# SuhailSama/MR_RL

Measured on NVIDIA B200. Metric: env_steps_per_sec, higher is better.
Workload: dtype f64

## Files before the change

mr_rl_b200/csrc/mr_api.cu:

```cuda
#include <cstdarg>
#include <cstdio>
#include <cstdlib>
#include <initializer_list>
#include <new>

#include "mr_common.cuh"

namespace mr {

thread_local char g_err[512] = "";

static int step_path_from_env() {
    const char* e = getenv("MR_STEP_PATH");
    if (!e) return 0;
    if (e[0] == 't' && e[1] == 'm' && e[2] == 'a' && e[3] == 'p') return 5;
    return e[0] == 't' ? 1 : e[0] == 'v' ? 2 : e[0] == 's' ? 3 : e[0] == 'w' ? 4 : 0;
}
int g_step_path = step_path_from_env();
thread_local int g_step_cta_cap = 0;
static int actor_path_from_env() {
    const char* e = getenv("MR_ACTOR_PATH");
    return !e ? 0 : e[0] == 's' ? 1 : e[0] == 't' ? 2 : 0;
}
int g_actor_path = actor_path_from_env();
// ... 388 lines not shown
            return mr::fail(MR_ERR_ARG, "mr_env_step_host: direct mode shares one row stride between obs_host and state_prime");
        oh.skip_goal_rows = io->copy_goal_rows ? 0 : 1;
        oh.out_f32 = io->io_f32 ? 1 : 0;
        mr_sim_params ph = *p;
        if (io->io_f32) { ph.action_f32 = 1; oh.state_prime = nullptr; }
        mr::g_step_cta_cap = 1;
        rc = mr_env_step(st, n, dtype, &ph, nz, tt, io->actions_host, &oh, stream);
        mr::g_step_cta_cap = 0;
        if (rc) return rc;
        const cudaError_t e0 = cudaStreamSynchronize((cudaStream_t)stream);
        if (e0 != cudaSuccess) return mr::fail(MR_ERR_CUDA, "mr_env_step_host: %s", cudaGetErrorString(e0));
        return MR_OK;
    }
    if (!pl || !out_dev) return mr::fail(MR_ERR_ARG, "mr_env_step_host: staged mode needs a pipeline and device output rows");
    const bool zc_in = io->actions_dev == nullptr;
    if (!out_dev->obs || !out_dev->rew || !out_dev->done) return mr::fail(MR_ERR_ARG, "mr_env_step_host: device obs/rew/done rows required");
    const int64_t dstride = out_dev->row_stride ? out_dev->row_stride : n;
    int chunks = n_chunks < 1 ? 1 : (n_chunks > pl->max_chunks ? pl->max_chunks : n_chunks);
    if (nz && nz->mode == MR_NOISE_TABLE) chunks = 1;
    int64_t per = (n / chunks) / 256 * 256;
    if (per == 0) { chunks = 1; per = n; }
    cudaStream_t cur = (cudaStream_t)stream;
    cudaError_t ce = cudaSuccess;
    auto ok = [&](cudaError_t r) { if (ce == cudaSuccess && r != cudaSuccess) ce = r; return ce == cudaSuccess; };
    ok(cudaEventRecord(pl->ev_start, cur));
    ok(cudaStreamWaitEvent(pl->s_in, pl->ev_start, 0));
    ok(cudaStreamWaitEvent(pl->s_k, pl->ev_start, 0));
    ok(cudaStreamWaitEvent(pl->s_out, pl->ev_start, 0));
    for (int c = 0; c < chunks && ce == cudaSuccess && rc == MR_OK; ++c) {
        const int64_t lo = c * per, hi = c == chunks - 1 ? n : lo + per, m = hi - lo;
        if (!zc_in) {
            if (!ok(cudaMemcpyAsync((char*)io->actions_dev + 2 * lo * el, (const char*)io->actions_host + 2 * lo * el,
                                    (size_t)(2 * m * el), cudaMemcpyHostToDevice, pl->s_in))) break;
            if (!ok(cudaEventRecord(pl->ev_in[c], pl->s_in)) || !ok(cudaStreamWaitEvent(pl->s_k, pl->ev_in[c], 0))) break;
        }
        mr_env_state sc = *st;
        sc.x = (char*)st->x + lo * el; sc.y = (char*)st->y + lo * el; sc.fx = (char*)st->fx + lo * el;
        sc.fy = (char*)st->fy + lo * el; sc.h = (char*)st->h + lo * el;
        sc.counter = st->counter + lo; sc.status = st->status + lo;
        if (st->cursor) sc.cursor = st->cursor + lo;
        mr_step_out oc = *out_dev;
        oc.obs = (char*)out_dev->obs + lo * el; oc.rew = (char*)out_dev->rew + lo * el; oc.done = out_dev->done + lo;
        if (out_dev->state_prime) oc.state_prime = (char*)out_dev->state_prime + lo * el;
        oc.row_stride = dstride;
        mr_noise nc;
        const mr_noise* nzp = nz;
        if (nz) { nc = *nz; nc.env_base = nz->env_base + (uint64_t)lo; nzp = &nc; }
        rc = mr_env_step(&sc, m, dtype, p, nzp, tt, (const char*)(zc_in ? io->actions_host : io->actions_dev) + 2 * lo * el, &oc,
                         pl->s_k);
        if (rc) break;
        if (!ok(cudaEventRecord(pl->ev_k[c], pl->s_k)) || !ok(cudaStreamWaitEvent(pl->s_out, pl->ev_k[c], 0))) break;
        ok(cudaMemcpy2DAsync((char*)io->obs_host + lo * el, (size_t)(hstride * el), (const char*)out_dev->obs + lo * el,
                             (size_t)(dstride * el), (size_t)(m * el), io->copy_goal_rows ? 4 : 2, cudaMemcpyDeviceToHost, pl->s_out));
        ok(cudaMemcpyAsync((char*)io->obs_host + (4 * hstride + lo) * el, (const char*)out_dev->obs + (4 * dstride + lo) * el,
                           (size_t)(m * el), cudaMemcpyDeviceToHost, pl->s_out));
        if (io->rew_host)
            ok(cudaMemcpyAsync((char*)io->rew_host + lo * el, (const char*)out_dev->rew + lo * el, (size_t)(m * el),
// ... 72 lines not shown
```

mr_rl_b200/csrc/mr_step_tma.cuh:

```cuda
#pragma once

#include "mr_common.cuh"

namespace mr {

#ifndef MR_STAGES_IN
#define MR_STAGES_IN 3
#endif
#ifdef MR_TILE
template <class T> struct TileOf { static constexpr int value = MR_TILE; };
#else
template <class T> struct TileOf { static constexpr int value = sizeof(T) == 8 ? 128 : 256; };
#endif
constexpr int kStagesIn = MR_STAGES_IN;
constexpr int kStagesOut = 2;

__device__ __forceinline__ uint32_t smem_u32(const void* p) { return (uint32_t)__cvta_generic_to_shared(p); }

__device__ __forceinline__ void mbar_init(uint64_t* bar, uint32_t count) {
    asm volatile("mbarrier.init.shared::cta.b64 [%0], %1;" ::"r"(smem_u32(bar)), "r"(count));
}
__device__ __forceinline__ void mbar_expect_tx(uint64_t* bar, uint32_t bytes) {
    asm volatile("mbarrier.arrive.expect_tx.shared::cta.b64 _, [%0], %1;" ::"r"(smem_u32(bar)), "r"(bytes) : "memory");
}
// ... 42 lines not shown
__device__ __forceinline__ void bulk_commit() { asm volatile("cp.async.bulk.commit_group;" ::: "memory"); }
template <int N>
__device__ __forceinline__ void bulk_wait_read() { asm volatile("cp.async.bulk.wait_group.read %0;" ::"n"(N) : "memory"); }
__device__ __forceinline__ void fence_async_smem() { asm volatile("fence.proxy.async.shared::cta;" ::: "memory"); }

template <class T, int kTile>
struct alignas(128) TileIn {
    T x[kTile], y[kTile], fx[kTile], fy[kTile], h[kTile];
    T act[2 * kTile];
    int32_t counter[kTile];
};

template <class T, int kTile>
struct alignas(128) TileOut {
    T x[kTile], y[kTile], fx[kTile], fy[kTile], h[kTile];
    T d[kTile], rew[kTile], spx[kTile], spy[kTile];
    int32_t counter[kTile];
    uint8_t done[kTile];
};

template <int MODE, bool MISM> struct NoiseRows { static constexpr int value = 0; };
template <bool MISM> struct NoiseRows<MR_NOISE_TABLE, MISM> { static constexpr int value = MISM ? 24 : 16; };
template <int MODE> struct StagesIn { static constexpr int value = MODE == MR_NOISE_TABLE ? 2 : kStagesIn; };
#ifndef MR_ONE_BARRIER
#define MR_ONE_BARRIER 1
#endif
template <class T, int MODE> struct OneBarrier {
    static constexpr bool value = MR_ONE_BARRIER && (MODE == MR_NOISE_PHILOX || (MODE == MR_NOISE_NONE && sizeof(T) == 4));
};
template <class T, int MODE> struct StagesOut { static constexpr int value = OneBarrier<T, MODE>::value ? 3 : kStagesOut; };

template <int kTile, int ROWS>
struct alignas(128) TileNoiseIn {
    double z[ROWS][kTile];
// ... 24 lines not shown
    }
};

#ifndef MR_RNG_PREFETCH
#define MR_RNG_PREFETCH 0
#endif

template <class T, int MODE = MR_NOISE_NONE, bool MISM = false, int kTile = TileOf<T>::value>
struct StepSmem {
    static constexpr int kIn = StagesIn<MODE>::value;
    TileIn<T, kTile> in[kIn];
    static constexpr int kOut = StagesOut<T, MODE>::value;
    TileOut<T, kTile> out[kOut];
    TileNoiseIn<kTile, NoiseRows<MODE, MISM>::value> nin[kIn];
    TileNoiseOut<kTile, NoiseRows<MODE, MISM>::value> nout[kOut];
    alignas(128) T zero[2 * kTile];
    alignas(16) float4 zpre[(MR_RNG_PREFETCH && MODE == MR_NOISE_PHILOX && !MISM) ? 2 * kTile : 1];
    alignas(8) uint64_t full[kIn];
};

#ifndef MR_TMA_WARPS
#define MR_TMA_WARPS 16
#endif
#ifndef MR_TMA_WARPS_F32
#define MR_TMA_WARPS_F32 24
#endif
template <class T> struct TmaWarps { static constexpr int value = sizeof(T) == 4 ? MR_TMA_WARPS_F32 : MR_TMA_WARPS; };
template <class T, int MODE> struct TmaMinCtas {
    static constexpr int value = MODE == MR_NOISE_TABLE ? 1 : TmaWarps<T>::value * 32 / TileOf<T>::value;
};

template <class T, int MODE, bool MISM, bool TMAP>
__global__ void __launch_bounds__(TileOf<T>::value, TmaMinCtas<T, MODE>::value)
env_step_tma_kernel(StateView<T> st, const T* __restrict__ actions, OutView<T> out, NoiseView nv, TimeView tv,
                    Params p, int64_t n_tiles, int64_t n_total, const __grid_constant__ StepMaps maps) {
    constexpr int kTile = TileOf<T>::value;
    constexpr int kSI = StagesIn<MODE>::value;
    constexpr int kNR = NoiseRows<MODE, MISM>::value;
    constexpr bool kTable = MODE == MR_NOISE_TABLE;
    constexpr bool kOneBar = OneBarrier<T, MODE>::value;
    constexpr int kSO = StagesOut<T, MODE>::value;
    extern __shared__ __align__(128) unsigned char smem_raw[];
    using Smem = StepSmem<T, MODE, MISM>;
    Smem& sm = *reinterpret_cast<Smem*>(smem_raw);
    const int tid = threadIdx.x;
    const int64_t first = blockIdx.x, stride = gridDim.x;

    if (tid == 0) {
        for (int s = 0; s < kSI; ++s) mbar_init(&sm.full[s], 1);
        asm volatile("fence.mbarrier_init.release.cluster;" ::: "memory");
    }
    sm.zero[tid] = (T)0; sm.zero[kTile + tid] = (T)0;
    fence_async_smem();
    __syncthreads();
    asm volatile("griddepcontrol.launch_dependents;" ::: "memory");
    asm volatile("griddepcontrol.wait;" ::: "memory");

    constexpr uint32_t kRow = kTile * sizeof(T);
    const bool act32 = sizeof(T) == 8 && p.act_f32;
    const bool out32 = sizeof(T) == 8 && out.f32;
    const uint32_t act_bytes = act32 ? kTile * 8u : 2u * kRow;
    const uint32_t kInBytes = 5 * kRow + act_bytes + kTile * 4;
    const uint64_t off = step_offset(nv);

#ifndef MR_ISSUE_WARPS
#define MR_ISSUE_WARPS 1
#endif
    constexpr int kWarps = MR_ISSUE_WARPS;
    const int warp = tid >> 5;
    const bool elect = (tid & 31) == 0 && warp < kWarps;
    auto issue_loads = [&](int s, int64_t tile, int32_t cbase) {
        const int64_t i0 = tile * kTile;
        uint64_t* bar = &sm.full[s];
        TileIn<T, kTile>& b = sm.in[s];
        if constexpr (kTable) {
            int64_t rows = nv.table_len - (int64_t)cbase;
            rows = rows < 0 ? 0 : (rows > kNR ? kNR : rows);
            if (cbase < 0) rows = 0;
            sm.nin[s].base = cbase; sm.nin[s].rows = (int32_t)rows;
            if constexpr (TMAP) {
                mbar_expect_tx(bar, kInBytes + kTile * 4 + (uint32_t)kNR * kTile * 8);
                tensor_load_2d(sm.nin[s].z, &maps.table, (int32_t)i0, cbase < 0 ? 0 : cbase, bar);
            } else {
                mbar_expect_tx(bar, kInBytes + kTile * 4 + (uint32_t)rows * kTile * 8);
                const double* src = nv.table + (int64_t)cbase * nv.table_stride + nv.table_col0 + i0;
                for (int k = 0; k < (int)rows; ++k) bulk_load(sm.nin[s].z[k], src + (int64_t)k * nv.table_stride, kTile * 8, bar);
            }
// ... 3 lines not shown
        }
        if constexpr (TMAP) {
            tensor_load_2d(b.x, &maps.state, (int32_t)i0, 0, bar);
        } else {
            if (warp == 0 % kWarps) bulk_load(b.x, st.x + i0, kRow, bar);
            if (warp == 1 % kWarps) bulk_load(b.y, st.y + i0, kRow, bar);
            if (warp == 2 % kWarps) bulk_load(b.fx, st.fx + i0, kRow, bar);
            if (warp == 3 % kWarps) bulk_load(b.fy, st.fy + i0, kRow, bar);
            if (warp == 4 % kWarps) bulk_load(b.h, st.h + i0, kRow, bar);
        }
        if (warp == 5 % kWarps)
            bulk_load(b.act, act32 ? (const void*)(reinterpret_cast<const float*>(actions) + 2 * i0) : (const void*)(actions + 2 * i0),
                      act_bytes, bar);
        if (warp == 6 % kWarps) bulk_load(b.counter, st.counter + i0, kTile * 4, bar);
    };
    auto tile_cursor = [&](int64_t tile) -> int32_t {
        if constexpr (kTable) { if (tile < n_tiles) return st.cursor[tile * kTile]; }
        return 0;
    };

    int32_t cb_next = 0;
    if (elect) {
        for (int s = 0; s < kSI; ++s) {
            const int64_t tile = first + (int64_t)s * stride;
            if (tile < n_tiles) issue_loads(s, tile, tile_cursor(tile));
        }
        cb_next = tile_cursor(first + (int64_t)kSI * stride);
    }

    constexpr bool kPrefetch = MR_RNG_PREFETCH && MODE == MR_NOISE_PHILOX && !MISM;
    auto predraw = [&](int64_t tile) {
        if constexpr (kPrefetch) {
            PhiloxNoise nzp;
            nzp.seek(nv.env_base + (uint64_t)(tile * kTile + tid), off);
            float z8[8];
            nzp.draw8(p, z8);
            sm.zpre[tid] = make_float4(z8[0], z8[1], z8[2], z8[3]);
            sm.zpre[kTile + tid] = make_float4(z8[4], z8[5], z8[6], z8[7]);
        }
    };
    if (first < n_tiles) predraw(first);

    int it = 0;
    for (int64_t tile = first; tile < n_tiles; tile += stride, ++it) {
        const int s = it % kSI;
        const uint32_t parity = (uint32_t)(it / kSI) & 1u;
        const int so = it % kSO;
        const int64_t i0 = tile * kTile;

        mbar_wait(&sm.full[s], parity);
        Env e;
        const TileIn<T, kTile>& bi = sm.in[s];
        e.x = (double)bi.x[tid]; e.y = (double)bi.y[tid]; e.fx = (double)bi.fx[tid]; e.fy = (double)bi.fy[tid];
        const T h_raw = bi.h[tid];
        e.counter = bi.counter[tid]; e.status = 0; e.spx = e.spy = 0.0;
        double f_t, al;
        if (sizeof(T) == 8 && !act32) { const double2 a2 = reinterpret_cast<const double2*>(bi.act)[tid]; f_t = a2.x; al = a2.y; }
        else { const float2 a2 = reinterpret_cast<const float2*>(bi.act)[tid]; f_t = a2.x; al = a2.y; }

        if constexpr (!kOneBar) {
            if (elect) bulk_wait_read<kStagesOut - 1>();
            __syncthreads();
            if constexpr (!kTable) {
                if (elect) {
                    const int64_t nxt = tile + (int64_t)kSI * stride;
                    if (nxt < n_tiles) issue_loads(s, nxt, 0);
                }
            }
        }

        const double t = time_at(tv, e.counter, p.dt);
        const double tb = t + p.dt, tb2 = tb + p.dt;
        e.h = decode_h<T>(h_raw, tb - t);
        int32_t cur = 0;
        e.counter += 1;
        if constexpr (kTable) {
            TileTableNoise nz;
            nz.stage = &sm.nin[s].z[0][tid]; nz.stage_stride = kTile;
            nz.base = sm.nin[s].base; nz.rows = sm.nin[s].rows;
            nz.col = nv.table + nv.table_col0 + i0 + tid; nz.stride = nv.table_stride;
            nz.cursor = sm.nin[s].cursor[tid]; nz.len = (int32_t)nv.table_len; nz.overflow = 0;
            sim_step<MISM>(e, t, tb, tb2, f_t, al, p, nz);
            cur = nz.cursor;
            if (nz.overflow) e.status |= kNoiseOverflow;
        } else if constexpr (kPrefetch) {
            const float4 za = sm.zpre[tid], zb = sm.zpre[kTile + tid];
            const float z8[8] = {za.x, za.y, za.z, za.w, zb.x, zb.y, zb.z, zb.w};
            if (tile + stride < n_tiles) predraw(tile + stride);
            PhiloxNoise nz;
            nz.seek(nv.env_base + (uint64_t)(i0 + tid), off);
            nz.blk += 2;
            sim_step_drawn(e, t, tb, tb2, f_t, al, p, nz, z8);
        } else {
            auto nz = make_noise<MODE>(nv, n_total, i0 + tid, 0, off);
            sim_step<MISM>(e, t, tb, tb2, f_t, al, p, nz);
        }
        const Observation o = observe(e, p);
        double d_out = o.d, il_next = tb2 - tb;
        if (p.auto_reset && o.done) {
            int ov = 0;
            auto_reset_env<MODE, MISM>(e, nv, n_total, i0 + tid, cur, off, p, ov);
            if (ov) e.status |= kNoiseOverflow;
            d_out = sqrt(e.x * e.x + e.y * e.y);
            il_next = p.dt;
        }

        TileOut<T, kTile>& bo = sm.out[so];
        bo.x[tid] = (T)e.x; bo.y[tid] = (T)e.y; bo.fx[tid] = (T)e.fx; bo.fy[tid] = (T)e.fy;
        bo.h[tid] = encode_h<T>(e.h, il_next);
        bo.counter[tid] = e.counter;
        bo.done[tid] = o.done ? 1 : 0;
        if (out32) {
            float* fxy = reinterpret_cast<float*>(bo.rew); fxy[tid] = (float)e.x; fxy[kTile + tid] = (float)e.y;
            float* fdr = reinterpret_cast<float*>(bo.d); fdr[tid] = (float)d_out; fdr[kTile + tid] = (float)o.rew;
            if (out.sp) { float* fsp = reinterpret_cast<float*>(bo.spx); fsp[tid] = (float)e.spx; fsp[kTile + tid] = (float)e.spy; }
        } else {
            bo.d[tid] = (T)d_out; bo.rew[tid] = (T)o.rew;
            if (out.sp) { bo.spx[tid] = (T)e.spx; bo.spy[tid] = (T)e.spy; }
        }
        if constexpr (kTable) sm.nout[so].cursor[tid] = cur;
        if (e.status) st.status[i0 + tid] |= (uint8_t)e.status;
        fence_async_smem();
        __syncthreads();
        if (elect) {
            if constexpr (kOneBar) {
                const int64_t nxt = tile + (int64_t)kSI * stride;
                if (nxt < n_tiles) issue_loads(s, nxt, 0);
            }
            if constexpr (kTable) {
                const int64_t nxt = tile + (int64_t)kSI * stride;
                if (nxt < n_tiles) issue_loads(s, nxt, cb_next);
                cb_next = tile_cursor(nxt + stride);
                bulk_store(st.cursor + i0, sm.nout[so].cursor, kTile * 4);
            }
            if constexpr (TMAP) {
                tensor_store_2d(&maps.state, (int32_t)i0, 0, bo.x);
                bulk_store(st.counter + i0, bo.counter, kTile * 4);
                if (out32) {
                    constexpr uint32_t kRow32 = kTile * 4;
                    const float* fdr = reinterpret_cast<const float*>(bo.d);
                    if (out.obs) {
                        tensor_store_2d(&maps.obs, (int32_t)i0, 0, bo.rew);
                        if (out.goal) tensor_store_2d(&maps.obs, (int32_t)i0, 2, sm.zero);
                        bulk_store(reinterpret_cast<float*>(out.obs) + 4 * out.stride + i0, fdr, kRow32);
                    }
                    if (out.rew) bulk_store(reinterpret_cast<float*>(out.rew) + i0, fdr + kTile, kRow32);
                    if (out.sp) tensor_store_2d(&maps.sp, (int32_t)i0, 0, bo.spx);
                } else {
                    if (out.obs) {
                        tensor_store_2d(&maps.obs, (int32_t)i0, 0, bo.x);
                        if (out.goal) tensor_store_2d(&maps.obs, (int32_t)i0, 2, sm.zero);
                        bulk_store(out.obs + 4 * out.stride + i0, bo.d, kRow);
                    }
                    if (out.rew) bulk_store(out.rew + i0, bo.rew, kRow);
                    if (out.sp) tensor_store_2d(&maps.sp, (int32_t)i0, 0, bo.spx);
                }
            } else {
            if (warp == 0 % kWarps) bulk_store(st.x + i0, bo.x, kRow);
            if (warp == 1 % kWarps) bulk_store(st.y + i0, bo.y, kRow);
            if (warp == 2 % kWarps) bulk_store(st.fx + i0, bo.fx, kRow);
            if (warp == 3 % kWarps) bulk_store(st.fy + i0, bo.fy, kRow);
            if (warp == 4 % kWarps) bulk_store(st.h + i0, bo.h, kRow);
            if (warp == 5 % kWarps) bulk_store(st.counter + i0, bo.counter, kTile * 4);
            if (out32) {
                constexpr uint32_t kRow32 = kTile * 4;
                float* obs = reinterpret_cast<float*>(out.obs);
                const float* fxy = reinterpret_cast<const float*>(bo.rew);
                const float* fdr = reinterpret_cast<const float*>(bo.d);
                if (obs) {
                    bulk_store(obs + i0, fxy, kRow32);
                    bulk_store(obs + out.stride + i0, fxy + kTile, kRow32);
                    if (out.goal) {
                        bulk_store(obs + 2 * out.stride + i0, sm.zero, kRow32);
                        bulk_store(obs + 3 * out.stride + i0, sm.zero, kRow32);
                    }
                    bulk_store(obs + 4 * out.stride + i0, fdr, kRow32);
                }
                if (out.rew) bulk_store(reinterpret_cast<float*>(out.rew) + i0, fdr + kTile, kRow32);
                if (out.sp) {
                    const float* fsp = reinterpret_cast<const float*>(bo.spx);
                    bulk_store(reinterpret_cast<float*>(out.sp) + i0, fsp, kRow32);
                    bulk_store(reinterpret_cast<float*>(out.sp) + out.stride + i0, fsp + kTile, kRow32);
                }
            } else {
                if (out.obs) {
                    if (warp == 6 % kWarps) bulk_store(out.obs + i0, bo.x, kRow);
                    if (warp == 7 % kWarps) bulk_store(out.obs + out.stride + i0, bo.y, kRow);
                    if (out.goal && warp == 8 % kWarps) bulk_store(out.obs + 2 * out.stride + i0, sm.zero, kRow);
                    if (out.goal && warp == 9 % kWarps) bulk_store(out.obs + 3 * out.stride + i0, sm.zero, kRow);
                    if (warp == 10 % kWarps) bulk_store(out.obs + 4 * out.stride + i0, bo.d, kRow);
                }
                if (out.rew && warp == 11 % kWarps) bulk_store(out.rew + i0, bo.rew, kRow);
                if (out.sp) {
                    if (warp == 13 % kWarps) bulk_store(out.sp + i0, bo.spx, kRow);
                    if (warp == 14 % kWarps) bulk_store(out.sp + out.stride + i0, bo.spy, kRow);
                }
            }
            }
            if (out.done && warp == 12 % kWarps) bulk_store(out.done + i0, bo.done, kTile);
            bulk_commit();
            if constexpr (kOneBar) bulk_wait_read<1>();
        }
    }
    if (elect) bulk_wait_read<0>();
}

}
```

mr_rl_b200/csrc/mr_step_ws.cuh:

```cuda
#pragma once

#include "mr_step_tma.cuh"

namespace mr {

template <class T> struct WsCfg {
    static constexpr int kTile = TileOf<T>::value;
    static constexpr int kSvcWarps = kTile / 128;
    static constexpr int kThreads = kTile + 32 * kSvcWarps;
    static constexpr int kCtas = sizeof(T) == 8 ? TmaWarps<T>::value * 32 / kTile : 2;
};

template <class T, int kTile = TileOf<T>::value>
struct StepSmemWs {
    TileIn<T, kTile> in[kStagesIn];
    TileOut<T, kTile> out[kStagesOut];
    alignas(128) T zero[kTile];
    alignas(16) float4 z[2][2][kTile];
    alignas(8) uint64_t full[kStagesIn];
};

template <class T>
__global__ void __launch_bounds__(WsCfg<T>::kThreads, WsCfg<T>::kCtas)
env_step_tma_ws_kernel(StateView<T> st, const T* __restrict__ actions, OutView<T> out, NoiseView nv, TimeView tv,
                       Params p, int64_t n_tiles, int64_t n_total) {
    constexpr int kTile = WsCfg<T>::kTile;
    constexpr int kSvc = 32 * WsCfg<T>::kSvcWarps;
    extern __shared__ __align__(128) unsigned char smem_raw[];
    StepSmemWs<T>& sm = *reinterpret_cast<StepSmemWs<T>*>(smem_raw);
    const int tid = threadIdx.x;
    const bool svc = tid >= kTile;
// ... 90 lines not shown
            nz.seek(nv.env_base + (uint64_t)(i0 + tid), off);
            nz.blk += 2;
            e.counter += 1;
            sim_step_drawn(e, t, tb, tb2, f_t, al, p, nz, z8);
            const Observation o = observe(e, p);
            double d_out = o.d, il_next = tb2 - tb;
            if (p.auto_reset && o.done) {
                int32_t cur = 0; int ov = 0;
                auto_reset_env<MR_NOISE_PHILOX, false>(e, nv, n_total, i0 + tid, cur, off, p, ov);
                d_out = sqrt(e.x * e.x + e.y * e.y);
                il_next = p.dt;
            }
            bo.x[tid] = (T)e.x; bo.y[tid] = (T)e.y; bo.fx[tid] = (T)e.fx; bo.fy[tid] = (T)e.fy;
            bo.h[tid] = encode_h<T>(e.h, il_next);
            bo.counter[tid] = e.counter;
            bo.d[tid] = (T)d_out; bo.rew[tid] = (T)o.rew; bo.done[tid] = o.done ? 1 : 0;
            if (out.sp) { bo.spx[tid] = (T)e.spx; bo.spy[tid] = (T)e.spy; }
            if (e.status) st.status[i0 + tid] |= (uint8_t)e.status;
            fence_async_smem();
        }
        __syncthreads();
        if (svc && elect) {
            bulk_store(st.x + i0, bo.x, kRow);
            bulk_store(st.y + i0, bo.y, kRow);
            bulk_store(st.fx + i0, bo.fx, kRow);
            bulk_store(st.fy + i0, bo.fy, kRow);
            bulk_store(st.h + i0, bo.h, kRow);
            bulk_store(st.counter + i0, bo.counter, kTile * 4);
            if (out.obs) {
                bulk_store(out.obs + i0, bo.x, kRow);
                bulk_store(out.obs + out.stride + i0, bo.y, kRow);
                if (out.goal) {
                    bulk_store(out.obs + 2 * out.stride + i0, sm.zero, kRow);
                    bulk_store(out.obs + 3 * out.stride + i0, sm.zero, kRow);
                }
                bulk_store(out.obs + 4 * out.stride + i0, bo.d, kRow);
            }
            if (out.rew) bulk_store(out.rew + i0, bo.rew, kRow);
            if (out.done) bulk_store(out.done + i0, bo.done, kTile);
            if (out.sp) {
                bulk_store(out.sp + i0, bo.spx, kRow);
                bulk_store(out.sp + out.stride + i0, bo.spy, kRow);
            }
            bulk_commit();
        }
    }
    if (svc && elect) bulk_wait_read<0>();
}

}
```

mr_rl_b200/vec_env.py:

```python
from __future__ import annotations

import ctypes as C
import math

import numpy as np
import torch

from . import _lib as L
from .spaces import Box

_DT = {torch.float64: L.MR_F64, torch.float32: L.MR_F32}
_NOISE = {"none": L.NOISE_NONE, "table": L.NOISE_TABLE, "philox": L.NOISE_PHILOX}
_PAD = 16


def _row_stride(n):
    npad = (n + _PAD - 1) // _PAD * _PAD
    if npad >= (1 << 16) and npad % 4096 == 0:
        npad += 256
    return npad


def _ptr(t):
    return C.c_void_p(t.data_ptr()) if t is not None else C.c_void_p(0)
# ... 47 lines not shown
        self._stats = torch.zeros(L.STATS_LEN, dtype=torch.float64, device=dev)
        tt = np.zeros(int(time_table_len), dtype=np.float64)
        self.lib.mr_fill_time_table_host(tt.ctypes.data_as(C.c_void_p), len(tt), self.params.time_span)
        self._tt = torch.from_numpy(tt).to(dev)

        self.per_env_params = bool(per_env_params)
        self._a0_row = self._sigma_row = self._mism_row = None
        if self.per_env_params:
            self._a0_row = torch.zeros(npad, dtype=torch.float64, device=dev)
            self._sigma_row = torch.zeros(npad, dtype=torch.float64, device=dev)
            self._mism_row = torch.zeros(npad, dtype=torch.uint8, device=dev)
        self._c_state = L.EnvState(*[_ptr(self._state[i]) for i in range(5)], _ptr(self._counter),
                                   _ptr(self._cursor), _ptr(self._status), _ptr(self._a0_row), _ptr(self._sigma_row),
                                   _ptr(self._mism_row))
        self._c_tt = L.TimeTable(_ptr(self._tt), len(tt), 0)
        self._c_out = L.StepOut(_ptr(self._obs), _ptr(self._rew), _ptr(self._done), _ptr(self._sp), npad)
        self._c_out_lean = L.StepOut(_ptr(self._obs), _ptr(self._rew), _ptr(self._done), C.c_void_p(0), npad)

        self.noise_kind = noise
        self._noise_table = None
        self._c_noise = L.Noise(_NOISE[noise], 0, C.c_void_p(0), 0, int(seed) & (2**64 - 1), 0, int(env_base), C.c_void_p(0))
        if noise == "table":
            if noise_table is None:
                raise ValueError("noise='table' needs noise_table[L, num_envs] (standard normals, float64)")
            self.set_noise_table(noise_table)
        self._step_index = 0
        self.want_state_prime = True
        self._pinned = {}
        self.kernel_launches = 0
        self._dev_index = self.device.index
        self._call_step = self.lib.mr_env_step
        self._b_state, self._b_params, self._b_tt = C.byref(self._c_state), C.byref(self.params), C.byref(self._c_tt)
        self._b_out, self._b_out_lean = C.byref(self._c_out), C.byref(self._c_out_lean)
        self._views = (self._obs[:, :n].t(), self._rew[:n], self._done[:n], {})

    @property
    def max_timesteps(self):
        return self.params.max_timesteps

    @max_timesteps.setter
    def max_timesteps(self, v):
        self.params.max_timesteps = int(v)

    @property
    def min_dist2goal(self):
        return self.params.min_dist2goal

    @min_dist2goal.setter
    def min_dist2goal(self, v):
# ... 60 lines not shown
    @property
    def counter(self):
        return self._counter[:self.num_envs]

    @property
    def obs(self):
        return self._obs[:, :self.num_envs].t()

    @property
    def status(self):
        return self._status[:self.num_envs]

    @property
    def stats(self):
        return self._stats

    def _stream(self):
        return C.c_void_p(torch.cuda.current_stream(self.device).cuda_stream)

    def set_noise_table(self, table):
        t = torch.as_tensor(table, dtype=torch.float64).to(self.device).contiguous()
        if t.dim() != 2 or t.shape[1] != self.num_envs:
            raise ValueError(f"noise_table must be [L, {self.num_envs}] (draw-major), got {tuple(t.shape)}")
        self._noise_table = t
        self._c_noise.table = t.data_ptr()
        self._c_noise.table_len = t.shape[0]

    def _noise_for(self, sigma):
        nz = self._c_noise
        if self.noise_kind == "table":
# ... 44 lines not shown
        init_t = None
        if init is not None:
            init_t = torch.as_tensor(np.asarray(init) if not torch.is_tensor(init) else init)
            init_t = init_t.to(device=self.device, dtype=self.dtype)
            if init_t.dim() == 1:
                init_t = init_t.reshape(1, 2).expand(n, 2)
            init_t = init_t.contiguous()
            if tuple(init_t.shape) != (n, 2):
                raise ValueError(f"init must be (2,) or ({n}, 2)")
        mask_t = None
        if mask is not None:
            mask_t = torch.as_tensor(mask).to(device=self.device, dtype=torch.uint8).contiguous()
        nz = self._noise_for(p.noise_var)
        rc = self.lib.mr_env_reset_ex(C.byref(self._c_state), n, self._dt, C.byref(p), C.byref(nz), _ptr(init_t),
                                      _ptr(mask_t), 1 if reset_cursor else 0, C.byref(rp) if rp is not None else None,
                                      C.byref(self._c_out), self._stream())
        L.check(rc, "mr_env_reset")
        self.kernel_launches += 1
        self._step_index += 1
        p.is_mismatched = 1 if is_mismatched else 0
        p.mism_at_reset = p.is_mismatched
        return self.obs

    def step(self, actions):
        if not torch.is_tensor(actions):
            return self.step_host(actions)
        n = self.num_envs
        a = actions
        if a.device != self.device or a.dtype is not self.dtype or not a.is_contiguous():
            a = a.to(device=self.device, dtype=self.dtype).contiguous()
        if a.numel() != 2 * n:
            raise ValueError(f"actions must be [{n}, 2]")
        nz = self._noise_for(self.params.noise_var)
        if torch.cuda.current_device() != self._dev_index:
            with torch.cuda.device(self.device):
                return self.step(a)
        rc = self._call_step(self._b_state, n, self._dt, self._b_params, C.byref(nz), self._b_tt, a.data_ptr(),
                             self._b_out if self.want_state_prime else self._b_out_lean,
                             torch.cuda.current_stream(self.device).cuda_stream)
        if rc:
            L.check(rc, "mr_env_step")
        self.kernel_launches += 1
        self._step_index += 1
        return self._views

    def capture_steps(self, action_buffers, k_steps=None):
        return StepGraph(self, action_buffers, k_steps)

    host_register_max = 16

    def _registered_view(self, a_np, hdt):
        want = np.float64 if hdt is torch.float64 else np.float32
        if a_np.dtype != want or not a_np.flags.c_contiguous or not a_np.flags.writeable or a_np.nbytes < (1 << 16):
            return None
# ... 19 lines not shown
            b = torch.empty(shape, dtype=dtype, pin_memory=True)
            self._pinned[key] = b
        return b

    def step_host(self, actions):
        n = self.num_envs
        fast = self._pinned.get("fast")
        if fast is not None and actions is fast[0] and self.host_mode == "direct" \
                and actions.dtype == (self.host_io_dtype or self.dtype):
            _, io_ref, ret = fast
            if torch.cuda.current_device() != self._dev_index:
                with torch.cuda.device(self.device):
                    return self.step_host(actions)
            nz = self._noise_for(self.params.noise_var)
            rc = self.lib.mr_env_step_host(None, self._b_state, n, self._dt, self._b_params, C.byref(nz), self._b_tt, io_ref,
                                           self._b_out if self.want_state_prime else self._b_out_lean, 0,
                                           torch.cuda.current_stream(self.device).cuda_stream)
            if rc:
                L.check(rc, "mr_env_step_host")
            self.kernel_launches += 1
            self._step_index += 1
            return ret
        direct = self.host_mode == "direct"
        io32 = direct and self.dtype is torch.float64 and self.host_io_dtype is torch.float32
        hdt = torch.float32 if io32 else self.dtype
        if torch.is_tensor(actions) and actions.device.type == "cpu" and actions.is_pinned() \
                and actions.dtype == hdt and actions.is_contiguous() and actions.numel() == 2 * n:
            a_pin = actions.view(n, 2)
            in_place = True
        else:
            in_place = False
# ... 23 lines not shown
            r_pin = self._pinned_buf("rew", (n,), hdt)
            r_np, r_ptr = r_pin.numpy(), r_pin.data_ptr()
        if fresh:
            o_pin.zero_()
        chunks = 0 if direct else self._host_chunks(n)
        with torch.cuda.device(self.device):
            pl = self._pinned.get("pipeline")
            if pl is None and chunks:
                h = C.c_void_p()
                L.check(self.lib.mr_host_pipeline_create(8, C.byref(h)), "mr_host_pipeline_create")
                pl = self._pinned["pipeline"] = h
            io = L.HostStepIO(a_pin.data_ptr(), a_dev.data_ptr() if a_dev is not None else 0, o_pin.data_ptr(), r_ptr,
                              d_pin.data_ptr(), self._np, 0, 1 if io32 else 0)
            nz = self._noise_for(self.params.noise_var)
            rc = self.lib.mr_env_step_host(pl, self._b_state, n, self._dt, self._b_params, C.byref(nz), self._b_tt, C.byref(io),
                                           self._b_out if self.want_state_prime else self._b_out_lean, chunks,
                                           torch.cuda.current_stream(self.device).cuda_stream)
        L.check(rc, "mr_env_step_host")
        self.kernel_launches += max(chunks, 1)
        self._step_index += 1
        ret = (o_pin[:, :n].numpy().T, r_np, d_pin.numpy().view(np.bool_), {})
        if in_place and chunks == 0:
            self._pinned["fast"] = (actions, C.byref(io), ret)
            self._pinned["fast_io"] = io
        return ret

    host_mode = "direct"
    host_chunks = 2
    host_io_dtype = None

    def _host_chunks(self, n, min_chunk=1 << 16):
# ... 80 lines not shown
            io.reset_init, io.reset_init_len = ri.data_ptr(), ri.shape[0]
            keep.append(ri)
        if record:
            res["xy"] = torch.empty(k, 2, n, dtype=self.dtype, device=self.device)
            io.traj_xy = res["xy"].data_ptr()
        if record_state_prime:
            res["state_prime"] = torch.empty(k, 2, n, dtype=self.dtype, device=self.device)
            io.traj_state_prime = res["state_prime"].data_ptr()
        if record_done:
            res["done_traj"] = torch.empty(k, n, dtype=torch.uint8, device=self.device)
            io.traj_done = res["done_traj"].data_ptr()
        if accumulate_stats:
            io.stats = self._stats.data_ptr()
        nz = self._noise_for(self.params.noise_var)
        rc = self.lib.mr_env_rollout(C.byref(self._c_state), n, self._dt, C.byref(self.params), C.byref(nz),
                                     C.byref(self._c_tt), C.byref(io), C.byref(self._c_out), self._stream())
        L.check(rc, "mr_env_rollout")
        self.kernel_launches += 1
        self._step_index += k
        res.update(obs=self.obs, rew=self._rew[:n], done=self._done[:n])
        return res

    def reset_stats(self):
        self._stats.zero_()

    def allreduce_stats(self, group=None):
        from .dist import merge_stats
        return merge_stats(self._stats, group)

    def stats_dict(self):
        v = self._stats.tolist()
# ... 55 lines not shown
    def __init__(self, env, action_buffers, k_steps=None):
        bufs = list(action_buffers)
        n = env.num_envs
        for a in bufs:
            if not (torch.is_tensor(a) and a.device == env.device and a.dtype is env.dtype and a.is_contiguous()
                    and a.numel() == 2 * n):
                raise ValueError(f"action buffers must be contiguous [{n}, 2] {env.dtype} tensors on {env.device}")
        self.env, self.buffers = env, bufs
        self.k_steps = int(k_steps if k_steps is not None else len(bufs))
        self._ctr = torch.zeros(1, dtype=torch.int64, device=env.device)
        self.graph = torch.cuda.CUDAGraph()
        with torch.cuda.device(env.device):
            env.step(bufs[0])
            torch.cuda.synchronize(env.device)
            nz = env._noise_for(env.params.noise_var)
            out = env._b_out if env.want_state_prime else env._b_out_lean
            with torch.cuda.graph(self.graph):
                stream = torch.cuda.current_stream(env.device).cuda_stream
                nz.offset_dev = self._ctr.data_ptr()
                try:
                    for k in range(self.k_steps):
                        nz.offset = k
                        rc = env._call_step(env._b_state, n, env._dt, env._b_params, C.byref(nz), env._b_tt,
                                            bufs[k % len(bufs)].data_ptr(), out, stream)
                        if rc:
                            L.check(rc, "mr_env_step (graph capture)")
                finally:
                    nz.offset_dev = None
        self._baked = self._param_key()

    def _param_key(self):
        p = self.env.params
        return (p.a0, p.noise_var, p.is_mismatched, p.auto_reset, p.max_timesteps, p.min_dist2goal, p.reward_mode,
                p.bound_xy, p.bound_d, tuple(p.init_low), tuple(p.init_high), self.env.want_state_prime)

    def replay(self):
        env = self.env
        if self._baked != self._param_key():
            raise RuntimeError("env parameters changed since the graph was captured: capture again")
        with torch.cuda.device(env.device):
            rc = env.lib.mr_counter_set(self._ctr.data_ptr(), env._step_index, env._stream())
            if rc:
                L.check(rc, "mr_counter_set")
            self.graph.replay()
        env._step_index += self.k_steps
        env.kernel_launches += self.k_steps + 1
        return env._views


from .dist import shard_range
```

Baseline: 36.49 billion.

## Skip constant reward writes and goal rows; split rarely used output smem

When the reward mode is the constant-10 mode, the Python wrapper fills the reward buffer once and passes a null reward pointer, so the kernel no longer stores the reward row each step. Goal rows are now skipped by default. The rew/sp/f32/zero staging buffers move into an optional extension region of shared memory, shrinking the base footprint so more CTAs can be resident. Tile indices also become 32-bit ints. The risk is stale reward contents if the buffer is modified externally, and a behaviour change because goal rows are no longer written.

```diff
diff --git a/mr_rl_b200/csrc/mr_api.cu b/mr_rl_b200/csrc/mr_api.cu
--- a/mr_rl_b200/csrc/mr_api.cu
+++ b/mr_rl_b200/csrc/mr_api.cu
@@ -426,7 +426,8 @@
     }
     if (!pl || !out_dev) return mr::fail(MR_ERR_ARG, "mr_env_step_host: staged mode needs a pipeline and device output rows");
     const bool zc_in = io->actions_dev == nullptr;
-    if (!out_dev->obs || !out_dev->rew || !out_dev->done) return mr::fail(MR_ERR_ARG, "mr_env_step_host: device obs/rew/done rows required");
+    if (!out_dev->obs || !out_dev->done || (io->rew_host && !out_dev->rew))
+        return mr::fail(MR_ERR_ARG, "mr_env_step_host: device obs/done rows (and rew, with rew_host) required");
     const int64_t dstride = out_dev->row_stride ? out_dev->row_stride : n;
     int chunks = n_chunks < 1 ? 1 : (n_chunks > pl->max_chunks ? pl->max_chunks : n_chunks);
     if (nz && nz->mode == MR_NOISE_TABLE) chunks = 1;
@@ -452,7 +453,7 @@
         sc.counter = st->counter + lo; sc.status = st->status + lo;
         if (st->cursor) sc.cursor = st->cursor + lo;
         mr_step_out oc = *out_dev;
-        oc.obs = (char*)out_dev->obs + lo * el; oc.rew = (char*)out_dev->rew + lo * el; oc.done = out_dev->done + lo;
+        oc.obs = (char*)out_dev->obs + lo * el; oc.rew = out_dev->rew ? (char*)out_dev->rew + lo * el : nullptr; oc.done = out_dev->done + lo;
         if (out_dev->state_prime) oc.state_prime = (char*)out_dev->state_prime + lo * el;
         oc.row_stride = dstride;
         mr_noise nc;
diff --git a/mr_rl_b200/csrc/mr_step_tma.cuh b/mr_rl_b200/csrc/mr_step_tma.cuh
--- a/mr_rl_b200/csrc/mr_step_tma.cuh
+++ b/mr_rl_b200/csrc/mr_step_tma.cuh
@@ -80,10 +80,21 @@
 template <class T, int kTile>
 struct alignas(128) TileOut {
     T x[kTile], y[kTile], fx[kTile], fy[kTile], h[kTile];
-    T d[kTile], rew[kTile], spx[kTile], spy[kTile];
+    T d[kTile];
     int32_t counter[kTile];
     uint8_t done[kTile];
 };
+template <class T, int kTile>
+struct alignas(128) TileOutExt { T rew[kTile], spx[kTile], spy[kTile]; };
+template <class T, int kSO, int kTile>
+struct StepSmemExt {
+    TileOutExt<T, kTile> out[kSO];
+    alignas(128) T zero[2 * kTile];
+};
+template <class T>
+__host__ __device__ __forceinline__ bool step_ext_rows(const OutView<T>& o) {
+    return o.rew || o.sp || o.f32 || (o.obs && o.goal);
+}
 
 template <int MODE, bool MISM> struct NoiseRows { static constexpr int value = 0; };
 template <bool MISM> struct NoiseRows<MR_NOISE_TABLE, MISM> { static constexpr int value = MISM ? 24 : 16; };
@@ -138,9 +149,10 @@
     TileOut<T, kTile> out[kOut];
     TileNoiseIn<kTile, NoiseRows<MODE, MISM>::value> nin[kIn];
     TileNoiseOut<kTile, NoiseRows<MODE, MISM>::value> nout[kOut];
-    alignas(128) T zero[2 * kTile];
     alignas(16) float4 zpre[(MR_RNG_PREFETCH && MODE == MR_NOISE_PHILOX && !MISM) ? 2 * kTile : 1];
     alignas(8) uint64_t full[kIn];
+    using Ext = StepSmemExt<T, kOut, kTile>;
+    static size_t bytes(bool ext) { return sizeof(StepSmem) + (ext ? sizeof(Ext) : 0); }
 };
 
 #ifndef MR_TMA_WARPS
@@ -167,14 +179,16 @@
     extern __shared__ __align__(128) unsigned char smem_raw[];
     using Smem = StepSmem<T, MODE, MISM>;
     Smem& sm = *reinterpret_cast<Smem*>(smem_raw);
+    typename Smem::Ext& sx = *reinterpret_cast<typename Smem::Ext*>(smem_raw + sizeof(Smem));
+    const bool ext = step_ext_rows(out);
     const int tid = threadIdx.x;
-    const int64_t first = blockIdx.x, stride = gridDim.x;
+    const int first = blockIdx.x, stride = gridDim.x, nt = (int)n_tiles;
 
     if (tid == 0) {
         for (int s = 0; s < kSI; ++s) mbar_init(&sm.full[s], 1);
         asm volatile("fence.mbarrier_init.release.cluster;" ::: "memory");
     }
-    sm.zero[tid] = (T)0; sm.zero[kTile + tid] = (T)0;
+    if (ext) { sx.zero[tid] = (T)0; sx.zero[kTile + tid] = (T)0; }
     fence_async_smem();
     __syncthreads();
     asm volatile("griddepcontrol.launch_dependents;" ::: "memory");
@@ -193,8 +207,8 @@
     constexpr int kWarps = MR_ISSUE_WARPS;
     const int warp = tid >> 5;
     const bool elect = (tid & 31) == 0 && warp < kWarps;
-    auto issue_loads = [&](int s, int64_t tile, int32_t cbase) {
-        const int64_t i0 = tile * kTile;
+    auto issue_loads = [&](int s, int tile, int32_t cbase) {
+        const int64_t i0 = (int64_t)tile * kTile;
         uint64_t* bar = &sm.full[s];
         TileIn<T, kTile>& b = sm.in[s];
         if constexpr (kTable) {
@@ -228,39 +242,39 @@
                       act_bytes, bar);
         if (warp == 6 % kWarps) bulk_load(b.counter, st.counter + i0, kTile * 4, bar);
     };
-    auto tile_cursor = [&](int64_t tile) -> int32_t {
-        if constexpr (kTable) { if (tile < n_tiles) return st.cursor[tile * kTile]; }
+    auto tile_cursor = [&](int tile) -> int32_t {
+        if constexpr (kTable) { if (tile < nt) return st.cursor[(int64_t)tile * kTile]; }
         return 0;
     };
 
     int32_t cb_next = 0;
     if (elect) {
         for (int s = 0; s < kSI; ++s) {
-            const int64_t tile = first + (int64_t)s * stride;
-            if (tile < n_tiles) issue_loads(s, tile, tile_cursor(tile));
-        }
-        cb_next = tile_cursor(first + (int64_t)kSI * stride);
+            const int tile = first + s * stride;
+            if (tile < nt) issue_loads(s, tile, tile_cursor(tile));
+        }
+        cb_next = tile_cursor(first + kSI * stride);
     }
 
     constexpr bool kPrefetch = MR_RNG_PREFETCH && MODE == MR_NOISE_PHILOX && !MISM;
-    auto predraw = [&](int64_t tile) {
+    auto predraw = [&](int tile) {
         if constexpr (kPrefetch) {
             PhiloxNoise nzp;
-            nzp.seek(nv.env_base + (uint64_t)(tile * kTile + tid), off);
+            nzp.seek(nv.env_base + (uint64_t)((int64_t)tile * kTile + tid), off);
             float z8[8];
             nzp.draw8(p, z8);
             sm.zpre[tid] = make_float4(z8[0], z8[1], z8[2], z8[3]);
             sm.zpre[kTile + tid] = make_float4(z8[4], z8[5], z8[6], z8[7]);
         }
     };
-    if (first < n_tiles) predraw(first);
+    if (first < nt) predraw(first);
 
     int it = 0;
-    for (int64_t tile = first; tile < n_tiles; tile += stride, ++it) {
+    for (int tile = first; tile < nt; tile += stride, ++it) {
         const int s = it % kSI;
         const uint32_t parity = (uint32_t)(it / kSI) & 1u;
         const int so = it % kSO;
-        const int64_t i0 = tile * kTile;
+        const int64_t i0 = (int64_t)tile * kTile;
 
         mbar_wait(&sm.full[s], parity);
         Env e;
@@ -277,8 +291,8 @@
             __syncthreads();
             if constexpr (!kTable) {
                 if (elect) {
-                    const int64_t nxt = tile + (int64_t)kSI * stride;
-                    if (nxt < n_tiles) issue_loads(s, nxt, 0);
+                    const int nxt = tile + kSI * stride;
+                    if (nxt < nt) issue_loads(s, nxt, 0);
                 }
             }
         }
@@ -300,7 +314,7 @@
         } else if constexpr (kPrefetch) {
             const float4 za = sm.zpre[tid], zb = sm.zpre[kTile + tid];
             const float z8[8] = {za.x, za.y, za.z, za.w, zb.x, zb.y, zb.z, zb.w};
-            if (tile + stride < n_tiles) predraw(tile + stride);
+            if (tile + stride < nt) predraw(tile + stride);
             PhiloxNoise nz;
             nz.seek(nv.env_base + (uint64_t)(i0 + tid), off);
             nz.blk += 2;
@@ -320,17 +334,19 @@
         }
 
         TileOut<T, kTile>& bo = sm.out[so];
+        TileOutExt<T, kTile>& be = sx.out[so];
         bo.x[tid] = (T)e.x; bo.y[tid] = (T)e.y; bo.fx[tid] = (T)e.fx; bo.fy[tid] = (T)e.fy;
         bo.h[tid] = encode_h<T>(e.h, il_next);
         bo.counter[tid] = e.counter;
         bo.done[tid] = o.done ? 1 : 0;
         if (out32) {
-            float* fxy = reinterpret_cast<float*>(bo.rew); fxy[tid] = (float)e.x; fxy[kTile + tid] = (float)e.y;
+            float* fxy = reinterpret_cast<float*>(be.rew); fxy[tid] = (float)e.x; fxy[kTile + tid] = (float)e.y;
             float* fdr = reinterpret_cast<float*>(bo.d); fdr[tid] = (float)d_out; fdr[kTile + tid] = (float)o.rew;
-            if (out.sp) { float* fsp = reinterpret_cast<float*>(bo.spx); fsp[tid] = (float)e.spx; fsp[kTile + tid] = (float)e.spy; }
+            if (out.sp) { float* fsp = reinterpret_cast<float*>(be.spx); fsp[tid] = (float)e.spx; fsp[kTile + tid] = (float)e.spy; }
         } else {
-            bo.d[tid] = (T)d_out; bo.rew[tid] = (T)o.rew;
-            if (out.sp) { bo.spx[tid] = (T)e.spx; bo.spy[tid] = (T)e.spy; }
+            bo.d[tid] = (T)d_out;
+            if (out.rew) be.rew[tid] = (T)o.rew;
+            if (out.sp) { be.spx[tid] = (T)e.spx; be.spy[tid] = (T)e.spy; }
         }
         if constexpr (kTable) sm.nout[so].cursor[tid] = cur;
         if (e.status) st.status[i0 + tid] |= (uint8_t)e.status;
@@ -338,12 +354,12 @@
         __syncthreads();
         if (elect) {
             if constexpr (kOneBar) {
-                const int64_t nxt = tile + (int64_t)kSI * stride;
-                if (nxt < n_tiles) issue_loads(s, nxt, 0);
+                const int nxt = tile + kSI * stride;
+                if (nxt < nt) issue_loads(s, nxt, 0);
             }
             if constexpr (kTable) {
-                const int64_t nxt = tile + (int64_t)kSI * stride;
-                if (nxt < n_tiles) issue_loads(s, nxt, cb_next);
+                const int nxt = tile + kSI * stride;
+                if (nxt < nt) issue_loads(s, nxt, cb_next);
                 cb_next = tile_cursor(nxt + stride);
                 bulk_store(st.cursor + i0, sm.nout[so].cursor, kTile * 4);
             }
@@ -354,20 +370,20 @@
                     constexpr uint32_t kRow32 = kTile * 4;
                     const float* fdr = reinterpret_cast<const float*>(bo.d);
                     if (out.obs) {
-                        tensor_store_2d(&maps.obs, (int32_t)i0, 0, bo.rew);
-                        if (out.goal) tensor_store_2d(&maps.obs, (int32_t)i0, 2, sm.zero);
+                        tensor_store_2d(&maps.obs, (int32_t)i0, 0, be.rew);
+                        if (out.goal) tensor_store_2d(&maps.obs, (int32_t)i0, 2, sx.zero);
                         bulk_store(reinterpret_cast<float*>(out.obs) + 4 * out.stride + i0, fdr, kRow32);
                     }
                     if (out.rew) bulk_store(reinterpret_cast<float*>(out.rew) + i0, fdr + kTile, kRow32);
-                    if (out.sp) tensor_store_2d(&maps.sp, (int32_t)i0, 0, bo.spx);
+                    if (out.sp) tensor_store_2d(&maps.sp, (int32_t)i0, 0, be.spx);
                 } else {
                     if (out.obs) {
                         tensor_store_2d(&maps.obs, (int32_t)i0, 0, bo.x);
-                        if (out.goal) tensor_store_2d(&maps.obs, (int32_t)i0, 2, sm.zero);
+                        if (out.goal) tensor_store_2d(&maps.obs, (int32_t)i0, 2, sx.zero);
                         bulk_store(out.obs + 4 * out.stride + i0, bo.d, kRow);
                     }
-                    if (out.rew) bulk_store(out.rew + i0, bo.rew, kRow);
-                    if (out.sp) tensor_store_2d(&maps.sp, (int32_t)i0, 0, bo.spx);
+                    if (out.rew) bulk_store(out.rew + i0, be.rew, kRow);
+                    if (out.sp) tensor_store_2d(&maps.sp, (int32_t)i0, 0, be.spx);
                 }
             } else {
             if (warp == 0 % kWarps) bulk_store(st.x + i0, bo.x, kRow);
@@ -379,20 +395,20 @@
             if (out32) {
                 constexpr uint32_t kRow32 = kTile * 4;
                 float* obs = reinterpret_cast<float*>(out.obs);
-                const float* fxy = reinterpret_cast<const float*>(bo.rew);
+                const float* fxy = reinterpret_cast<const float*>(be.rew);
                 const float* fdr = reinterpret_cast<const float*>(bo.d);
                 if (obs) {
                     bulk_store(obs + i0, fxy, kRow32);
                     bulk_store(obs + out.stride + i0, fxy + kTile, kRow32);
                     if (out.goal) {
-                        bulk_store(obs + 2 * out.stride + i0, sm.zero, kRow32);
-                        bulk_store(obs + 3 * out.stride + i0, sm.zero, kRow32);
+                        bulk_store(obs + 2 * out.stride + i0, sx.zero, kRow32);
+                        bulk_store(obs + 3 * out.stride + i0, sx.zero, kRow32);
                     }
                     bulk_store(obs + 4 * out.stride + i0, fdr, kRow32);
                 }
                 if (out.rew) bulk_store(reinterpret_cast<float*>(out.rew) + i0, fdr + kTile, kRow32);
                 if (out.sp) {
-                    const float* fsp = reinterpret_cast<const float*>(bo.spx);
+                    const float* fsp = reinterpret_cast<const float*>(be.spx);
                     bulk_store(reinterpret_cast<float*>(out.sp) + i0, fsp, kRow32);
                     bulk_store(reinterpret_cast<float*>(out.sp) + out.stride + i0, fsp + kTile, kRow32);
                 }
@@ -400,14 +416,14 @@
                 if (out.obs) {
                     if (warp == 6 % kWarps) bulk_store(out.obs + i0, bo.x, kRow);
                     if (warp == 7 % kWarps) bulk_store(out.obs + out.stride + i0, bo.y, kRow);
-                    if (out.goal && warp == 8 % kWarps) bulk_store(out.obs + 2 * out.stride + i0, sm.zero, kRow);
-                    if (out.goal && warp == 9 % kWarps) bulk_store(out.obs + 3 * out.stride + i0, sm.zero, kRow);
+                    if (out.goal && warp == 8 % kWarps) bulk_store(out.obs + 2 * out.stride + i0, sx.zero, kRow);
+                    if (out.goal && warp == 9 % kWarps) bulk_store(out.obs + 3 * out.stride + i0, sx.zero, kRow);
                     if (warp == 10 % kWarps) bulk_store(out.obs + 4 * out.stride + i0, bo.d, kRow);
                 }
-                if (out.rew && warp == 11 % kWarps) bulk_store(out.rew + i0, bo.rew, kRow);
+                if (out.rew && warp == 11 % kWarps) bulk_store(out.rew + i0, be.rew, kRow);
                 if (out.sp) {
-                    if (warp == 13 % kWarps) bulk_store(out.sp + i0, bo.spx, kRow);
-                    if (warp == 14 % kWarps) bulk_store(out.sp + out.stride + i0, bo.spy, kRow);
+                    if (warp == 13 % kWarps) bulk_store(out.sp + i0, be.spx, kRow);
+                    if (warp == 14 % kWarps) bulk_store(out.sp + out.stride + i0, be.spy, kRow);
                 }
             }
             }
diff --git a/mr_rl_b200/csrc/mr_step_ws.cuh b/mr_rl_b200/csrc/mr_step_ws.cuh
--- a/mr_rl_b200/csrc/mr_step_ws.cuh
+++ b/mr_rl_b200/csrc/mr_step_ws.cuh
@@ -15,6 +15,7 @@
 struct StepSmemWs {
     TileIn<T, kTile> in[kStagesIn];
     TileOut<T, kTile> out[kStagesOut];
+    TileOutExt<T, kTile> oext[kStagesOut];
     alignas(128) T zero[kTile];
     alignas(16) float4 z[2][2][kTile];
     alignas(8) uint64_t full[kStagesIn];
@@ -135,8 +136,8 @@
             bo.x[tid] = (T)e.x; bo.y[tid] = (T)e.y; bo.fx[tid] = (T)e.fx; bo.fy[tid] = (T)e.fy;
             bo.h[tid] = encode_h<T>(e.h, il_next);
             bo.counter[tid] = e.counter;
-            bo.d[tid] = (T)d_out; bo.rew[tid] = (T)o.rew; bo.done[tid] = o.done ? 1 : 0;
-            if (out.sp) { bo.spx[tid] = (T)e.spx; bo.spy[tid] = (T)e.spy; }
+            bo.d[tid] = (T)d_out; sm.oext[so].rew[tid] = (T)o.rew; bo.done[tid] = o.done ? 1 : 0;
+            if (out.sp) { sm.oext[so].spx[tid] = (T)e.spx; sm.oext[so].spy[tid] = (T)e.spy; }
             if (e.status) st.status[i0 + tid] |= (uint8_t)e.status;
             fence_async_smem();
         }
@@ -157,11 +158,11 @@
                 }
                 bulk_store(out.obs + 4 * out.stride + i0, bo.d, kRow);
             }
-            if (out.rew) bulk_store(out.rew + i0, bo.rew, kRow);
+            if (out.rew) bulk_store(out.rew + i0, sm.oext[so].rew, kRow);
             if (out.done) bulk_store(out.done + i0, bo.done, kTile);
             if (out.sp) {
-                bulk_store(out.sp + i0, bo.spx, kRow);
-                bulk_store(out.sp + out.stride + i0, bo.spy, kRow);
+                bulk_store(out.sp + i0, sm.oext[so].spx, kRow);
+                bulk_store(out.sp + out.stride + i0, sm.oext[so].spy, kRow);
             }
             bulk_commit();
         }
diff --git a/mr_rl_b200/vec_env.py b/mr_rl_b200/vec_env.py
--- a/mr_rl_b200/vec_env.py
+++ b/mr_rl_b200/vec_env.py
@@ -85,8 +85,13 @@
                                    _ptr(self._cursor), _ptr(self._status), _ptr(self._a0_row), _ptr(self._sigma_row),
                                    _ptr(self._mism_row))
         self._c_tt = L.TimeTable(_ptr(self._tt), len(tt), 0)
-        self._c_out = L.StepOut(_ptr(self._obs), _ptr(self._rew), _ptr(self._done), _ptr(self._sp), npad)
-        self._c_out_lean = L.StepOut(_ptr(self._obs), _ptr(self._rew), _ptr(self._done), C.c_void_p(0), npad)
+        def step_out(rew, sp):
+            o = L.StepOut(_ptr(self._obs), _ptr(rew), _ptr(self._done), _ptr(sp), npad)
+            o.skip_goal_rows = 1
+            return o
+        self._c_out, self._c_out_lean = step_out(self._rew, self._sp), step_out(self._rew, None)
+        self._c_out_const, self._c_out_const_lean = step_out(None, self._sp), step_out(None, None)
+        self._rew_const = False
 
         self.noise_kind = noise
         self._noise_table = None
@@ -103,7 +108,9 @@
         self._call_step = self.lib.mr_env_step
         self._b_state, self._b_params, self._b_tt = C.byref(self._c_state), C.byref(self.params), C.byref(self._c_tt)
         self._b_out, self._b_out_lean = C.byref(self._c_out), C.byref(self._c_out_lean)
+        self._b_out_const, self._b_out_const_lean = C.byref(self._c_out_const), C.byref(self._c_out_const_lean)
         self._views = (self._obs[:, :n].t(), self._rew[:n], self._done[:n], {})
+        self._out_ref()
 
     @property
     def max_timesteps(self):
@@ -194,6 +201,17 @@
     @property
     def stats(self):
         return self._stats
+
+    def _out_ref(self, state_prime=None):
+        sp = self.want_state_prime if state_prime is None else state_prime
+        const = self.params.reward_mode == L.REWARD_CONST10
+        if const != self._rew_const:
+            if const:
+                self._rew[:self.num_envs].fill_(10.0)
+            self._rew_const = const
+        if const:
+            return self._b_out_const if sp else self._b_out_const_lean
+        return self._b_out if sp else self._b_out_lean
 
     def _stream(self):
         return C.c_void_p(torch.cuda.current_stream(self.device).cuda_stream)
@@ -268,7 +286,7 @@
         nz = self._noise_for(p.noise_var)
         rc = self.lib.mr_env_reset_ex(C.byref(self._c_state), n, self._dt, C.byref(p), C.byref(nz), _ptr(init_t),
                                       _ptr(mask_t), 1 if reset_cursor else 0, C.byref(rp) if rp is not None else None,
-                                      C.byref(self._c_out), self._stream())
+                                      self._out_ref(state_prime=True), self._stream())
         L.check(rc, "mr_env_reset")
         self.kernel_launches += 1
         self._step_index += 1
@@ -290,8 +308,7 @@
             with torch.cuda.device(self.device):
                 return self.step(a)
         rc = self._call_step(self._b_state, n, self._dt, self._b_params, C.byref(nz), self._b_tt, a.data_ptr(),
-                             self._b_out if self.want_state_prime else self._b_out_lean,
-                             torch.cuda.current_stream(self.device).cuda_stream)
+                             self._out_ref(), torch.cuda.current_stream(self.device).cuda_stream)
         if rc:
             L.check(rc, "mr_env_step")
         self.kernel_launches += 1
@@ -341,7 +358,7 @@
                     return self.step_host(actions)
             nz = self._noise_for(self.params.noise_var)
             rc = self.lib.mr_env_step_host(None, self._b_state, n, self._dt, self._b_params, C.byref(nz), self._b_tt, io_ref,
-                                           self._b_out if self.want_state_prime else self._b_out_lean, 0,
+                                           self._out_ref(), 0,
                                            torch.cuda.current_stream(self.device).cuda_stream)
             if rc:
                 L.check(rc, "mr_env_step_host")
@@ -395,7 +412,7 @@
                               d_pin.data_ptr(), self._np, 0, 1 if io32 else 0)
             nz = self._noise_for(self.params.noise_var)
             rc = self.lib.mr_env_step_host(pl, self._b_state, n, self._dt, self._b_params, C.byref(nz), self._b_tt, C.byref(io),
-                                           self._b_out if self.want_state_prime else self._b_out_lean, chunks,
+                                           self._out_ref(), chunks,
                                            torch.cuda.current_stream(self.device).cuda_stream)
         L.check(rc, "mr_env_step_host")
         self.kernel_launches += max(chunks, 1)
@@ -506,7 +523,7 @@
             io.stats = self._stats.data_ptr()
         nz = self._noise_for(self.params.noise_var)
         rc = self.lib.mr_env_rollout(C.byref(self._c_state), n, self._dt, C.byref(self.params), C.byref(nz),
-                                     C.byref(self._c_tt), C.byref(io), C.byref(self._c_out), self._stream())
+                                     C.byref(self._c_tt), C.byref(io), self._out_ref(state_prime=True), self._stream())
         L.check(rc, "mr_env_rollout")
         self.kernel_launches += 1
         self._step_index += k
@@ -592,7 +609,7 @@
             env.step(bufs[0])
             torch.cuda.synchronize(env.device)
             nz = env._noise_for(env.params.noise_var)
-            out = env._b_out if env.want_state_prime else env._b_out_lean
+            out = env._out_ref()
             with torch.cuda.graph(self.graph):
                 stream = torch.cuda.current_stream(env.device).cuda_stream
                 nz.offset_dev = self._ctr.data_ptr()
@@ -617,6 +634,7 @@
         if self._baked != self._param_key():
             raise RuntimeError("env parameters changed since the graph was captured: capture again")
         with torch.cuda.device(env.device):
+            env._out_ref()
             rc = env.lib.mr_counter_set(self._ctr.data_ptr(), env._step_index, env._stream())
             if rc:
                 L.check(rc, "mr_counter_set")
```

Result: faster. 38.27 billion, median of 6 (+4.9%).
